# tylerlum/Vine_Robot_IsaacGymEnvs

Measured on NVIDIA B200. Metric: env-steps/s (whole box, device-timed), higher is better.
Workload: dtype f32

## Files before the change

### vine_robot_isaacgymenvs_b200/csrc/vine_b200.cu

```cuda
#include <cuda_runtime.h>
#include <stdio.h>
#include <stdlib.h>

#include "vine_device.cuh"
#include "vine_launch.cuh"

#define VINE_BLOCK 128
#ifndef VINE_STEP_MIN_BLOCKS
#define VINE_STEP_MIN_BLOCKS 0
#endif
#ifndef VINE_STEP_MIN_BLOCKS_CONTACT
#define VINE_STEP_MIN_BLOCKS_CONTACT 12
#endif
#define VINE_DBG_W 28

struct StepArgs {
  int64_t n, gid0;
  int64_t first, end;
  uint32_t k0, k1;
  float4 *S0, *S1, *S2, *S3, *S4, *S5;
  float2* ring;
  uint32_t* ctr;
  const float2* actions;
  float* obs; float* obs_clamped; float* rew;
// ... 186 lines not shown
  const bool noisy = p.randomize && p.obs_noise != 0.f;
  if (noisy) {
#pragma unroll
    for (uint32_t b = 0; b < VINE_MAX_OBS / 4; ++b) {
      if ((int)(4 * b) < p.O) normal4(philox4x32(a.k0, a.k1, E.gid, VINE_SITE_OBS_NOISE, E.step, b), &noise[4 * b]);
    }
  }
  PostOut o;
  post_physics(p, in, noisy ? noise : nullptr, o);
  agg = __fadd_rn(agg, o.rew);

  a.S0[e] = make_float4(q[0], q[1], q[2], q[3]);
  a.S1[e] = make_float4(q[4], q[5], qd[0], qd[1]);
  a.S2[e] = make_float4(qd[2], qd[3], qd[4], qd[5]);
  a.S3[e] = make_float4(E.smoothed, E.prev_cart_vel, E.prev_err, E.lip);
  a.S4[e] = make_float4(tip_y, tip_z, cart_body_vy, agg);
  if (E.reset_in) a.S5[e] = make_float4(target[1], target[2], obj[0], obj[1]);
  if (p.D > 0) a.ring[(int64_t)(E.step % (uint32_t)p.D) * a.n + e] = make_float2(E.new_rail, E.new_fpam);
  a.ctr[e] = E.step + 1u;
  a.rew[e] = o.rew;
  a.reset[e] = o.reset;
  a.progress[e] = progress;
  a.timeout[e] = o.timeout;
#pragma unroll
  for (int i = 0; i < VINE_MAX_OBS; ++i) if (i < p.O) row[i] = o.obs[i];
  if (a.dbg) {
    float* dbg = a.dbg + e * VINE_DBG_W;
    dbg[0] = E.u_rail; dbg[1] = E.u_fpam; dbg[2] = in.prev_u_rail; dbg[3] = E.rail_force;
    dbg[4] = tipvel_y; dbg[5] = tipvel_z;
    dbg[19] = cart_y_body;
#pragma unroll
    for (int i = 0; i < VINE_NUM_REWARDS; ++i) dbg[6 + i] = o.r[i];
#pragma unroll
    for (int i = 0; i < 6; ++i) dbg[20 + i] = div_rn(__fsub_rn(in.q[i], in.prev_q[i]), p.control_dt);
    dbg[26] = div_rn(__fsub_rn(in.tip[1], in.prev_tip[1]), p.control_dt);
    dbg[27] = div_rn(__fsub_rn(in.tip[2], in.prev_tip[2]), p.control_dt);
  }
}

#ifndef VINE_BLOCK_CONTACT
#define VINE_BLOCK_CONTACT 32
#endif

__device__ __forceinline__ void store_obs_rows_scattered(const VineParams& p, const StepArgs& a, const float* s_obs, int64_t mine) {
  const int lane = threadIdx.x & 31, w0 = threadIdx.x & ~31;
#pragma unroll 1
  for (int r = 0; r < 32; ++r) {
    const int64_t er = __shfl_sync(0xffffffffu, mine, r);
    if (er >= 0 && lane < p.O) {
      const float v = s_obs[(w0 + r) * (VINE_MAX_OBS + 1) + lane];
      a.obs[er * p.O + lane] = v;
      if (a.obs_clamped) a.obs_clamped[er * p.O + lane] = fminf(fmaxf(v, -p.clip_obs), p.clip_obs);
    }
  }
}

__device__ __forceinline__ int64_t slot_env(const StepArgs& a, int64_t slot) {
  if (!a.list) return a.first + slot;
  return (int64_t)(a.list_reversed ? a.list[a.n - 1 - slot] : a.list[slot]);
}

template <bool CONTACT>
__global__ void __launch_bounds__(CONTACT ? VINE_BLOCK_CONTACT : VINE_BLOCK, CONTACT ? VINE_STEP_MIN_BLOCKS_CONTACT : VINE_STEP_MIN_BLOCKS)
vine_step_kernel(const __grid_constant__ VineParams p, const StepArgs a) {
  vine_launch::grid_dependency_sync();
  constexpr int BLOCK = CONTACT ? VINE_BLOCK_CONTACT : VINE_BLOCK;
  __shared__ float s_obs[BLOCK * (VINE_MAX_OBS + 1)];
  __shared__ ContactScratch s_contact[CONTACT ? BLOCK / 32 : 1];
  ContactScratch* cs = &s_contact[CONTACT ? threadIdx.x >> 5 : 0];
  const int64_t count = a.list_count ? (int64_t)*a.list_count : a.end - a.first;
  const int lanes = (CONTACT && a.list && count <= (int64_t)gridDim.x * 8) ? 8 : BLOCK;
#pragma unroll 1
  for (int64_t base = (int64_t)blockIdx.x * lanes; base < count; base += (int64_t)gridDim.x * lanes) {
    const int64_t slot = base + threadIdx.x;
    const bool live = slot < count && (int)threadIdx.x < lanes;
    const bool ghost = CONTACT && !live;
    const int64_t e = live ? slot_env(a, slot) : (ghost ? slot_env(a, base) : -1);
    if (live || ghost) {
      EnvStep E; Dyn d;
      env_begin(p, a, e, E, d);
      Obstacles ob = {0, -1, 0.f, 0.f, 0.f, 0.f};
      ContactCache cc = {0u, ghost ? -1e30f : 1e30f, 0u};
      if (CONTACT) { const float4 s5 = a.S5[e]; build_obstacles(p, s5.x, s5.y, s5.z, s5.w, cs, ob); }
      const float m00inv = rcp_approx(fmaf(p.h, p.damping, p.mtot));
#pragma unroll 1
      for (int i = 0; i < p.C; ++i) {
        JointImp J;
        env_sim_step_begin(p, a, i, E, d, J);
#pragma unroll 1
        for (int s = 0; s < p.S; ++s) substep<CONTACT>(p, J, m00inv, E.rail_force, ob, cs, cc, d, E.lip, ghost);
      }
      if (!ghost) {
        env_end(p, a, e, E, d, s_obs + threadIdx.x * (VINE_MAX_OBS + 1));
        if (CONTACT && a.near) a.near[e] = cc.seen != 0u;
      }
    }
    __syncthreads();
    if (CONTACT && a.list) store_obs_rows_scattered(p, a, s_obs, live ? e : -1);
    else store_obs_block<BLOCK>(s_obs, p.O, a.first + base - (int64_t)blockIdx.x * BLOCK, a.end, p.clip_obs, a.obs, a.obs_clamped);
    __syncthreads();
  }
}

__global__ void __launch_bounds__(VINE_BLOCK) vine_step_far_kernel(const __grid_constant__ VineParams p, const StepArgs a) {
  __shared__ float s_obs[VINE_BLOCK * (VINE_MAX_OBS + 1)];
  const int64_t count = a.list_count ? a.n - (int64_t)*a.list_count : a.n;
  const int64_t slot = (int64_t)blockIdx.x * VINE_BLOCK + threadIdx.x;
  if ((int64_t)blockIdx.x * VINE_BLOCK >= count) return;
  const bool live = slot < count;
  int64_t e = live ? slot_env(a, slot) : -1;
  if (live) {
    EnvStep E; Dyn d;
    env_begin(p, a, e, E, d);
    Obstacles ob;
    { const float4 s5 = a.S5[e]; obstacle_bbox(p, s5.x, s5.y, s5.z, s5.w, ob); }
    float gap = chain_obstacle_gap(p, ob, d);
    bool given_up = !(gap > 0.f);
    float disp = -gap;
    ContactCache cc = {0u, 0.f, 0u};
    const float m00inv = rcp_approx(fmaf(p.h, p.damping, p.mtot));
#pragma unroll 1
    for (int i = 0; i < p.C && !given_up; ++i) {
      JointImp J;
      env_sim_step_begin(p, a, i, E, d, J);
#pragma unroll 1
      for (int s = 0; s < p.S; ++s) {
        substep<false>(p, J, m00inv, E.rail_force, ob, nullptr, cc, d, E.lip);
        disp += chain_displacement_bound(p, d);
        if (disp > p.cull_slack) {
          gap = chain_obstacle_gap(p, ob, d);
          if (!(gap > 0.f)) { given_up = true; break; }
          disp = -gap;
        }
      }
      E.lip = 0.f;
    }
    if (given_up) {
      a.redo_list[atomicAdd(a.redo_count, 1)] = (int32_t)e;
      e = -1;
    } else {
      env_end(p, a, e, E, d, s_obs + threadIdx.x * (VINE_MAX_OBS + 1));
      a.near[e] = 0;
    }
  }
  __syncthreads();
  store_obs_rows_scattered(p, a, s_obs, e);
}

__global__ void __launch_bounds__(1024) vine_bin_kernel(const StepArgs a) {
  __shared__ int s_near[32], s_far[32], s_base[2];
  const int64_t e = (int64_t)blockIdx.x * 1024 + threadIdx.x;
  const bool valid = e < a.n, nr = valid && a.near[e] != 0;
  const unsigned bn = __ballot_sync(0xffffffffu, nr), bf = __ballot_sync(0xffffffffu, valid && !nr);
  const int lane = threadIdx.x & 31, warp = threadIdx.x >> 5;
  if (lane == 0) { s_near[warp] = __popc(bn); s_far[warp] = __popc(bf); }
  __syncthreads();
  if (warp == 0) {
    const int cn = s_near[lane], cf = s_far[lane];
    int in = cn, jf = cf;
#pragma unroll
    for (int off = 1; off < 32; off <<= 1) {
      const int tn = __shfl_up_sync(0xffffffffu, in, off), tf = __shfl_up_sync(0xffffffffu, jf, off);
      if (lane >= off) { in += tn; jf += tf; }
    }
    s_near[lane] = in - cn; s_far[lane] = jf - cf;
    if (lane == 31) { s_base[0] = atomicAdd(a.bin_cursor, in); s_base[1] = atomicAdd(a.bin_cursor + 1, jf); }
  }
  __syncthreads();
  if (!valid) return;
  const unsigned lt = (1u << lane) - 1u;
  if (nr) a.perm[s_base[0] + s_near[warp] + __popc(bn & lt)] = (int32_t)e;
  else a.perm[a.n - 1 - (s_base[1] + s_far[warp] + __popc(bf & lt))] = (int32_t)e;
}

__global__ void vine_init_kernel(const __grid_constant__ VineParams p, const StepArgs a) {
  const int64_t e = (int64_t)blockIdx.x * blockDim.x + threadIdx.x;
  if (e >= a.n) return;
  uint32_t u[12];
  for (uint32_t b = 0; b < 3; ++b) {
    const uint4 r = philox4x32(a.k0, a.k1, (uint32_t)(a.gid0 + e), VINE_SITE_RESET, 0x40000000u, b);
    u[4 * b] = r.x; u[4 * b + 1] = r.y; u[4 * b + 2] = r.z; u[4 * b + 3] = r.w;
  }
  float target[3]; sample_targets(p, u, target);
  const float4 z = make_float4(0.f, 0.f, 0.f, 0.f);
  a.S0[e] = z; a.S1[e] = z; a.S2[e] = z; a.S3[e] = z;
  a.S4[e] = make_float4(p.tip0_y, p.tip0_z, 0.f, 0.f);
  a.S5[e] = make_float4(target[1], target[2], 0.f, 0.f);
  for (int k = 0; k < p.D; ++k) a.ring[(int64_t)k * a.n + e] = make_float2(0.f, 0.f);
  a.ctr[e] = 0u;
}

__global__ void vine_reset_idx_kernel(const __grid_constant__ VineParams p, const StepArgs a, const int64_t* ids, int64_t n_ids) {
  const int64_t i = (int64_t)blockIdx.x * blockDim.x + threadIdx.x;
  if (i >= n_ids) return;
  const int64_t e = ids[i];
  if (e < 0 || e >= a.n) return;
  float q[6], qd[6], target[3], obj[2];
  const float4 s5 = a.S5[e];
  target[0] = 0.f; target[1] = s5.x; target[2] = s5.y; obj[0] = s5.z; obj[1] = s5.w;
  reset_env(p, a.k0, a.k1, (uint32_t)(a.gid0 + e), a.ctr[e] | 0x80000000u, q, qd, target, obj);
  float4 s3 = a.S3[e], s4 = a.S4[e];
  s3.z = 0.f;
  s4.w = 0.f;
  if (!p.stale) {
    Dyn d; rel_to_abs(q, qd, d);
    float vy, vz; tip_fk(d, s4.x, s4.y, vy, vz);
    s4.z = 0.f; s3.w = 0.f; s3.y = 0.f;
  }
  a.S0[e] = make_float4(q[0], q[1], q[2], q[3]);
  a.S1[e] = make_float4(q[4], q[5], 0.f, 0.f);
// ... 80 lines not shown
  in.u_rail = io.u_rail_velocity[e]; in.prev_u_rail = io.prev_u_rail_velocity[e];
  for (int i = 0; i < VINE_MAX_CFI; ++i) in.contact[i] = (io.contact_force_norms && i < p.C) ? io.contact_force_norms[(int64_t)i * n + e] : 0.f;
  in.reset_in = io.reset_buf_in[e]; in.progress = io.progress_buf[e];
  float noise[VINE_MAX_OBS];
  const bool noisy = p.randomize && io.obs_noise != nullptr;
  if (noisy) for (int i = 0; i < p.O; ++i) noise[i] = io.obs_noise[(int64_t)p.O * e + i];
  PostOut o;
  post_physics(p, in, noisy ? noise : nullptr, o);
  for (int i = 0; i < p.O; ++i) io.obs_buf[(int64_t)p.O * e + i] = o.obs[i];
  io.rew_buf[e] = o.rew;
  if (io.reward_matrix) for (int i = 0; i < VINE_NUM_REWARDS; ++i) io.reward_matrix[VINE_NUM_REWARDS * e + i] = o.r[i];
  io.reset_buf_out[e] = o.reset;
  io.timeout_buf[e] = o.timeout;
}

__global__ void vine_pre_physics_kernel(const __grid_constant__ VineParams p, int64_t n, const VinePrePhysicsIO io) {
  const int64_t e = (int64_t)blockIdx.x * blockDim.x + threadIdx.x;
  if (e >= n) return;
  float a0 = io.actions[2 * e], a1 = io.actions[2 * e + 1];
  if (p.randomize && io.action_noise) {
    a0 = __fadd_rn(a0, __fmul_rn(p.act_noise, io.action_noise[2 * e]));
    a1 = __fadd_rn(a1, __fmul_rn(p.act_noise, io.action_noise[2 * e + 1]));
  }
  float u_rail, u_fpam;
  rescale_actions(p, a0, a1, u_rail, u_fpam);
  if (p.D > 0) {
    const float* hi = io.history_in + (int64_t)2 * p.D * e;
    float* ho = io.history_out + (int64_t)2 * p.D * e;
    const float o_rail = hi[0], o_fpam = hi[1];
    for (int k = 0; k + 1 < p.D; ++k) { ho[2 * k] = hi[2 * k + 2]; ho[2 * k + 1] = hi[2 * k + 3]; }
    ho[2 * (p.D - 1)] = u_rail; ho[2 * (p.D - 1) + 1] = u_fpam;
    u_rail = o_rail; u_fpam = o_fpam;
  }
  float s = io.smoothed_in[e];
  apply_overrides_and_smooth(p, u_rail, u_fpam, s);
  io.u_rail_velocity[e] = u_rail; io.u_fpam[e] = u_fpam; io.smoothed_out[e] = s;
}

__global__ void vine_actuation_kernel(const __grid_constant__ VineParams p, int64_t n, const VineActuationIO io) {
  const int64_t e = (int64_t)blockIdx.x * blockDim.x + threadIdx.x;
  if (e >= n) return;
  JointLaw law; joint_law_unscaled(law);
  if (io.dynamics_scaling) {
    const float* s = io.dynamics_scaling + 20 * e;
    for (int j = 0; j < VINE_NL; ++j) {
      law.K[j] = __fmul_rn(law.K[j], s[4 * j]); law.Cd[j] = __fmul_rn(law.Cd[j], s[4 * j + 1]);
      law.b[j] = __fmul_rn(law.b[j], s[4 * j + 2]); law.B[j] = __fmul_rn(law.B[j], s[4 * j + 3]);
    }
  }
  float pv = io.prev_cart_vel[e], pe = io.prev_cart_vel_error[e];
  io.dof_efforts[6 * e] = rail_controller(p, io.cart_vel_y[e], io.u_rail_velocity[e],
                                          io.accel_scaling ? io.accel_scaling[e] : 1.f, pv, pe);
  for (int j = 0; j < VINE_NL; ++j)
    io.dof_efforts[6 * e + j + 1] = joint_torque(law, j, io.dof_pos[6 * e + j + 1], io.dof_vel[6 * e + j + 1], io.u_fpam_to_use[e]);
  io.prev_cart_vel_out[e] = pv; io.prev_cart_vel_error_out[e] = pe;
}

template <bool CONTACT>
__global__ void __launch_bounds__(VINE_BLOCK) vine_simulate_kernel(const __grid_constant__ VineParams p, int64_t n, const VineSimulateIO io) {
  __shared__ ContactScratch s_contact[CONTACT ? VINE_BLOCK / 32 : 1];
  ContactScratch* cs = &s_contact[CONTACT ? threadIdx.x >> 5 : 0];
  const int64_t e0 = (int64_t)blockIdx.x * blockDim.x + threadIdx.x;
  const bool ghost = e0 >= n;
  if (ghost && !CONTACT) return;
  const int64_t e = ghost ? n - 1 : e0;
  float q[6], qd[6], efforts[6];
  for (int i = 0; i < 6; ++i) { q[i] = io.dof_pos[6 * e + i]; qd[i] = io.dof_vel[6 * e + i]; efforts[i] = io.dof_efforts[6 * e + i]; }
  JointLaw law; joint_law_unscaled(law);
  if (io.dynamics_scaling) {
    const float* s = io.dynamics_scaling + 20 * e;
    for (int j = 0; j < VINE_NL; ++j) {
      law.K[j] = __fmul_rn(law.K[j], s[4 * j]); law.Cd[j] = __fmul_rn(law.Cd[j], s[4 * j + 1]);
      law.b[j] = __fmul_rn(law.b[j], s[4 * j + 2]); law.B[j] = __fmul_rn(law.B[j], s[4 * j + 3]);
    }
  }
  const float u_use = io.u_fpam_to_use ? io.u_fpam_to_use[e] : 0.f;
  Obstacles ob = {0, -1, 0.f, 0.f, 0.f, 0.f};
  ContactCache cc = {0u, ghost ? -1e30f : 1e30f, 0u};
  if (CONTACT) build_obstacles(p, io.target_positions[3 * e + 1], io.target_positions[3 * e + 2],
                               io.object_info[2 * e], io.object_info[2 * e + 1], cs, ob);
  Dyn d; rel_to_abs(q, qd, d);
  JointImp J; joint_implicit_consts(p, law, u_use, efforts, J);
  float lip = 0.f;
  const float m00inv = rcp_approx(fmaf(p.h, p.damping, p.mtot));
#pragma unroll 1
  for (int s = 0; s < p.S; ++s) substep<CONTACT>(p, J, m00inv, efforts[0], ob, cs, cc, d, lip, ghost);
  if (ghost) return;
  float ty, tz, vy, vz; tip_fk(d, ty, tz, vy, vz);
  abs_to_rel(d, q, qd);
  for (int i = 0; i < 6; ++i) { io.dof_pos[6 * e + i] = q[i]; io.dof_vel[6 * e + i] = qd[i]; }
  if (io.tip_positions) { io.tip_positions[3 * e] = 0.f; io.tip_positions[3 * e + 1] = ty; io.tip_positions[3 * e + 2] = tz; }
  if (io.tip_velocities) { io.tip_velocities[3 * e] = 0.f; io.tip_velocities[3 * e + 1] = vy; io.tip_velocities[3 * e + 2] = vz; }
  if (io.shelf_contact_force) io.shelf_contact_force[e] = lip;
}

__global__ void vine_philox_kernel(uint32_t k0, uint32_t k1, uint32_t gid, uint32_t site, uint32_t step, uint32_t block0,
                                   int64_t n_blocks, uint32_t* out) {
  const int64_t i = (int64_t)blockIdx.x * blockDim.x + threadIdx.x;
  if (i >= n_blocks) return;
  const uint4 r = philox4x32(k0, k1, gid, site, step, block0 + (uint32_t)i);
  out[4 * i] = r.x; out[4 * i + 1] = r.y; out[4 * i + 2] = r.z; out[4 * i + 3] = r.w;
}

__global__ void vine_gae_kernel(const float* __restrict__ rewards, const float* __restrict__ values,
                                const float* __restrict__ dones, const float* __restrict__ last_values,
                                const float* __restrict__ last_dones, int64_t T, int64_t N, float gamma, float gt,
                                float* __restrict__ adv, float* __restrict__ ret) {
  vine_launch::grid_dependency_sync();
  const int64_t e = (int64_t)blockIdx.x * blockDim.x + threadIdx.x;
  if (e >= N) return;
  float nextv = last_values[e], nonterm = __fsub_rn(1.0f, last_dones[e]), lastgaelam = 0.f;
  float r = rewards[(T - 1) * N + e], v = values[(T - 1) * N + e], dn = dones[(T - 1) * N + e];
  for (int64_t t = T - 1; t >= 0; --t) {
    float r2 = 0.f, v2 = 0.f, d2 = 0.f;
    if (t > 0) { r2 = rewards[(t - 1) * N + e]; v2 = values[(t - 1) * N + e]; d2 = dones[(t - 1) * N + e]; }
    const float delta = __fsub_rn(__fadd_rn(r, __fmul_rn(__fmul_rn(gamma, nextv), nonterm)), v);
    lastgaelam = __fadd_rn(delta, __fmul_rn(__fmul_rn(gt, nonterm), lastgaelam));
    adv[t * N + e] = lastgaelam;
    ret[t * N + e] = __fadd_rn(lastgaelam, v);
    nextv = v; nonterm = __fsub_rn(1.0f, dn);
    r = r2; v = v2; dn = d2;
  }
}

static inline unsigned grid_for(int64_t n, int block) { return (unsigned)((n + block - 1) / block); }

extern "C" {

int vine_abi_version(void) { return VINE_ABI_VERSION; }

int vine_set_programmatic_launch(int enabled) {
  const int before = vine_launch::programmatic_launch_enabled();
  vine_launch::programmatic_launch_enabled() = enabled ? 1 : 0;
  return before;
}

int vine_config_defaults(VineConfig* c) {
  if (!c) return VINE_ERR_INVALID_ARG;
  memset(c, 0, sizeof(*c));
  c->struct_size = (int32_t)sizeof(*c);
  c->substeps = 10; c->dt = 0.00833; c->gravity_z = -9.81;
  c->control_freq_inv = 4; c->max_episode_length = 500;
  c->clip_observations = 5.0; c->clip_actions = 1.0;
  c->observation_type = VINE_OBS_POS_AND_FD_VEL_AND_OBJ_INFO; c->scale_observations = 1;
  c->create_shelf = 0; c->create_pipe = 1;
  c->use_smoothed_fpam = 1; c->action_delay = 1;
  c->smoothing_alpha_inflate = 0.81; c->smoothing_alpha_deflate = 0.86;
  c->fpam_min = -0.1; c->fpam_max = 3.0; c->rail_velocity_scale = 1.0;
  c->damping = 2e-2; c->stiffness = 0.0;
  c->rail_soft_limit = 0.3; c->rail_p_gain = 10.0; c->rail_d_gain = 0.0; c->rail_acceleration = 8.0;
  c->randomize_dof_init = 1; c->randomize_targets = 1;
  c->random_init_cart_min_y = -0.1 * 0.3; c->random_init_cart_max_y = 0.3;
  c->success_dist = 0.08;
  c->min_target_depth_in_obstacle = -0.05; c->max_target_depth_in_obstacle = 0.2;
  c->min_target_y = -0.48; c->max_target_y = -0.4; c->min_target_z = 0.58; c->max_target_z = 0.67;
  const double w[VINE_NUM_REWARDS] = {0, 0, 1, 0, 0.1, 0, 0, 0, 0, 1, 0, 0, 0.10};
  memcpy(c->reward_weights, w, sizeof(w));
  c->use_target_reached_reset = 1;
  c->vine_randomize = 1;
  c->dynamics_scaling_min = 0.999; c->dynamics_scaling_max = 1.001;
  c->accel_target_scaling_min = 1.0; c->accel_target_scaling_max = 1.0;
  c->torque_law_integration = VINE_TORQUE_LAW_IMPLICIT;
  c->emulate_stale_body_state = 1;
  c->revolute_lower = -3.4e38; c->revolute_upper = 3.4e38;
  c->prismatic_lower = -3.4e38; c->prismatic_upper = 3.4e38;
  c->contact_stiffness = 2000.0; c->contact_damping = 2.0; c->contact_rest_offset = 0.001;
  c->contact_cull_slack = 0.01; c->contact_binning = 1;
  return VINE_OK;
}
// ... 350 lines not shown
```

### vine_robot_isaacgymenvs_b200/csrc/vine_device.cuh

```cuda
#pragma once
#include <cuda_runtime.h>

#include "vine_params.h"

#define VDEV __device__ __forceinline__

VDEV uint4 philox4x32(uint32_t k0, uint32_t k1, uint32_t c0, uint32_t c1, uint32_t c2, uint32_t c3) {
#pragma unroll
  for (int r = 0; r < 10; ++r) {
    const uint32_t hi0 = __umulhi(0xD2511F53u, c0), lo0 = 0xD2511F53u * c0;
    const uint32_t hi1 = __umulhi(0xCD9E8D57u, c2), lo1 = 0xCD9E8D57u * c2;
    c0 = hi1 ^ c1 ^ k0; c1 = lo1; c2 = hi0 ^ c3 ^ k1; c3 = lo0;
    k0 += 0x9E3779B9u; k1 += 0xBB67AE85u;
  }
  return make_uint4(c0, c1, c2, c3);
}

VDEV float rcp_approx(float x) { float r; asm("rcp.approx.ftz.f32 %0, %1;" : "=f"(r) : "f"(x)); return r; }
VDEV float sin_approx(float x) { float r; asm("sin.approx.ftz.f32 %0, %1;" : "=f"(r) : "f"(x)); return r; }
VDEV float cos_approx(float x) { float r; asm("cos.approx.ftz.f32 %0, %1;" : "=f"(r) : "f"(x)); return r; }
VDEV float div_rn(float a, float b) {
  const bool bypass = a == 0.f && fabsf(b) > 0.f && fabsf(b) < __int_as_float(0x7f800000);
  const float q = __fdiv_rn(bypass ? 1.f : a, b);
  return bypass ? __int_as_float(__float_as_int(a) ^ (__float_as_int(b) & (int)0x80000000)) : q;
// ... 305 lines not shown
#pragma unroll
    for (int j = 0; j < VINE_NL; ++j) {
      const float lw = VINE_LINK_LEN * d.v[j + 1];
      vy = fmaf(-lw, d.C[j], vy); vz = fmaf(-lw, d.S[j], vz);
      ch[32 * (CH_PY + j + 1)] = py[j + 1]; ch[32 * (CH_PZ + j + 1)] = pz[j + 1];
      ch[32 * (CH_VY + j + 1)] = vy; ch[32 * (CH_VZ + j + 1)] = vz;
      ch[32 * (CH_S + j)] = d.S[j]; ch[32 * (CH_C + j)] = d.C[j]; ch[32 * (CH_W + j)] = d.v[j + 1];
    }
  }
  const int cnt = __popc(pm);
  const unsigned below = (1u << lane) - 1u;
  int next = 0, total = 0;
#pragma unroll
  for (int k = 0; k < 5; ++k) {
    const unsigned plane = __ballot_sync(0xffffffffu, (cnt >> k) & 1);
    next += __popc(plane & below) << k;
    total += __popc(plane) << k;
  }
  unsigned todo = pm, toadd = pm;
  int next_add = next;
  float lfy = 0.f, lfz = 0.f;
#pragma unroll 1
  for (int base = 0; base < total; base += VINE_PAIR_PASS) {
    while (todo && next < base + VINE_PAIR_PASS) {
      const int b = __ffs(todo) - 1;
      todo &= todo - 1;
      cs->item[next - base] = (unsigned short)(lane | (b << 5));
      ++next;
    }
    __syncwarp();
    const int n_pass = min(VINE_PAIR_PASS, total - base);
#pragma unroll 1
    for (int i = lane; i < n_pass; i += 32) {
      const int it = cs->item[i];
      PairLoad L;
      pair_load(p, cs, it & 31, it >> 5, L);
      cs->res[i][0] = L.fy; cs->res[i][1] = L.fz; cs->res[i][2] = L.t;
    }
    __syncwarp();
    while (toadd && next_add < base + VINE_PAIR_PASS) {
      const int b = __ffs(toadd) - 1;
      toadd &= toadd - 1;
      const float* rs = cs->res[next_add - base];
      ++next_add;
      const float Lfy = rs[0], Lfz = rs[1], Lt = rs[2];
      if (Lfy != 0.f || Lfz != 0.f) {
        const int r = b / 5, j = b - 5 * r;
        f[0] += Lfy;
#pragma unroll
        for (int m = 0; m < VINE_NL; ++m) {
          const float q = m == j ? Lt : (py[m + 1] - py[m]) * Lfz - (pz[m + 1] - pz[m]) * Lfy;
          if (m <= j) f[m + 1] += q;
        }
        if (r == ob.lip) { lfy -= Lfy; lfz -= Lfz; }
      }
    }
    __syncwarp();
  }
  const float l2 = lfy * lfy + lfz * lfz;
  const float l = sqrtf(l2 > 0.f ? l2 : 1.f);
  return l2 > 0.f ? l : 0.f;
}

struct JointImp { float kk[VINE_NL], ek[VINE_NL], tc[VINE_NL], gam[VINE_NL], diag[VINE_NL]; };

VDEV void joint_implicit_consts(const VineParams& p, const JointLaw& law, float u_use, const float efforts[6], JointImp& J) {
#pragma unroll
  for (int j = 0; j < VINE_NL; ++j) {
    float dd;
    if (p.implicit_law) {
      J.kk[j] = p.stiffness + law.K[j]; dd = p.damping + law.Cd[j];
      J.tc[j] = -fmaf(law.B[j], u_use, law.b[j]);
    } else {
      J.kk[j] = p.stiffness; dd = p.damping; J.tc[j] = efforts[j + 1];
    }
    J.ek[j] = fmaf(p.h, J.kk[j], dd);
    J.gam[j] = fmaf(p.h, dd, p.h * p.h * J.kk[j]) + p.armature;
  }
#pragma unroll
  for (int j = 0; j < VINE_NL; ++j) J.diag[j] = p.alpha[j] + J.gam[j] + (j + 1 < VINE_NL ? J.gam[j + 1] : 0.f);
}

template <bool CONTACT>
VDEV void substep(const VineParams& p, const JointImp& J, float m00inv, float rail_force, const Obstacles& ob,
                  ContactScratch* cs, ContactCache& cc, Dyn& d, float& lip, bool ghost = false) {
  float a[VINE_NL], b[VINE_NL], As[VINE_NL], Bs[VINE_NL];
#pragma unroll
  for (int j = 0; j < VINE_NL; ++j) { const float w2 = __fmul_rn(d.v[j + 1], d.v[j + 1]); a[j] = __fmul_rn(d.C[j], w2); b[j] = __fmul_rn(d.S[j], w2); }
  As[VINE_NL - 2] = __fmul_rn(p.Lbeta[VINE_NL - 1], a[VINE_NL - 1]);
  Bs[VINE_NL - 2] = __fmul_rn(p.Lbeta[VINE_NL - 1], b[VINE_NL - 1]);
#pragma unroll
  for (int j = VINE_NL - 3; j >= 0; --j) {
    As[j] = __fmaf_rn(p.Lbeta[j + 1], a[j + 1], As[j + 1]);
    Bs[j] = __fmaf_rn(p.Lbeta[j + 1], b[j + 1], Bs[j + 1]);
  }
  float f[6];
  f[0] = __fmaf_rn(-p.inv_L, __fmaf_rn(p.Lbeta[0], b[0], Bs[0]), __fmaf_rn(-p.damping, d.v[0], rail_force));
  {
    float Ap = a[0], Bp = b[0];
    f[1] = __fmaf_rn(d.C[0], Bs[0], __fmul_rn(d.S[0], __fsub_rn(p.gbeta[0], As[0])));
#pragma unroll
    for (int j = 1; j < VINE_NL; ++j) {
      const float P = j == VINE_NL - 1 ? __fmul_rn(p.Lbeta[j], Ap) : __fmaf_rn(p.Lbeta[j], Ap, As[j]);
      const float Q = j == VINE_NL - 1 ? __fmul_rn(p.Lbeta[j], Bp) : __fmaf_rn(p.Lbeta[j], Bp, Bs[j]);
      f[j + 1] = __fmaf_rn(d.C[j], Q, __fmul_rn(d.S[j], __fsub_rn(p.gbeta[j], P)));
      if (j + 1 < VINE_NL) { Ap = __fadd_rn(Ap, a[j]); Bp = __fadd_rn(Bp, b[j]); }
    }
  }
  {
    float tn = 0.f;
#pragma unroll
    for (int j = VINE_NL - 1; j >= 0; --j) {
      const float th = j == 0 ? d.x[1] : __fsub_rn(d.x[j + 1], d.x[j]);
      const float thd = j == 0 ? d.v[1] : __fsub_rn(d.v[j + 1], d.v[j]);
      const float t = __fmaf_rn(-J.ek[j], thd, __fmaf_rn(-J.kk[j], th, J.tc[j]));
      f[j + 1] = __fadd_rn(f[j + 1], j == VINE_NL - 1 ? t : __fsub_rn(t, tn));
      tn = t;
    }
  }
  if constexpr (CONTACT) lip = contact_forces(p, ob, cs, cc, d, f, ghost);
  float M[6][6];
#pragma unroll
  for (int j = 0; j < VINE_NL; ++j) {
    M[j + 1][0] = __fmul_rn(-p.beta[j], d.C[j]);
    M[j + 1][j + 1] = J.diag[j];
#pragma unroll
    for (int m = 0; m < j; ++m) {
      const float c = __fmaf_rn(d.C[j], d.C[m], __fmul_rn(d.S[j], d.S[m]));
      M[j + 1][m + 1] = (m == j - 1) ? __fmaf_rn(p.Lbeta[j], c, -J.gam[j]) : __fmul_rn(p.Lbeta[j], c);
    }
  }
  float dinv[6];
  dinv[0] = m00inv;
#pragma unroll
  for (int j = 1; j < 6; ++j) {
    float u[5];
    float dj = M[j][j];
#pragma unroll
    for (int q = 0; q < j; ++q) {
      float uq = M[j][q];
#pragma unroll
      for (int r = 0; r < q; ++r) uq = __fmaf_rn(-u[r], M[q][r], uq);
      u[q] = uq;
      const float l = __fmul_rn(uq, dinv[q]);
      M[j][q] = l;
      dj = __fmaf_rn(-uq, l, dj);
    }
    dinv[j] = rcp_approx(dj);
  }
#pragma unroll
  for (int i = 1; i < 6; ++i)
#pragma unroll
    for (int q = 0; q < i; ++q) f[i] = __fmaf_rn(-M[i][q], f[q], f[i]);
#pragma unroll
  for (int i = 0; i < 6; ++i) f[i] = __fmul_rn(f[i], dinv[i]);
#pragma unroll
  for (int i = 4; i >= 0; --i)
#pragma unroll
    for (int q = i + 1; q < 6; ++q) f[i] = __fmaf_rn(-M[q][i], f[q], f[i]);
  d.v[0] = __fmaf_rn(p.h, f[0], d.v[0]); d.x[0] = __fmaf_rn(p.h, d.v[0], d.x[0]);
#pragma unroll
  for (int j = 0; j < VINE_NL; ++j) {
    d.v[j + 1] = __fmaf_rn(p.h, f[j + 1], d.v[j + 1]);
    d.x[j + 1] = __fmaf_rn(p.h, d.v[j + 1], d.x[j + 1]);
    link_trig(d.x[j + 1], d.S[j], d.C[j]);
  }
}

VDEV float norm3_torch(float x, float y, float z) {
  return __fsqrt_rn(__fmaf_rn(z, z, __fmaf_rn(y, y, __fmul_rn(x, x))));
}

struct PostIn {
  float q[6], qd[6], prev_q[6];
  float tip[3], prev_tip[3], tipvel[3], target[3], target_vel[3], obj[2];
  float cart_y, smoothed, u_fpam, u_rail, prev_u_rail;
  float contact[VINE_MAX_CFI];
  int64_t reset_in, progress;
};

struct PostOut { float obs[VINE_MAX_OBS]; float rew; float r[VINE_NUM_REWARDS]; int64_t reset; unsigned char timeout; };

VDEV void observation_row(const VineParams& p, const PostIn& in, float raw[VINE_MAX_OBS]) {
  float fdq[6], fdt[3];
#pragma unroll
  for (int i = 0; i < 6; ++i) fdq[i] = div_rn(__fsub_rn(in.q[i], in.prev_q[i]), p.control_dt);
#pragma unroll
  for (int i = 0; i < 3; ++i) fdt[i] = div_rn(__fsub_rn(in.tip[i], in.prev_tip[i]), p.control_dt);
  const int t = p.obs_type;
#pragma unroll
  for (int i = 0; i < VINE_MAX_OBS; ++i) raw[i] = 0.f;
  if (t == VINE_OBS_TIP_AND_CART_AND_OBJ_INFO) {
    raw[0] = in.q[0]; raw[1] = fdq[0];
#pragma unroll
    for (int i = 0; i < 3; ++i) { raw[2 + i] = in.tip[i]; raw[5 + i] = fdt[i]; raw[8 + i] = in.target[i]; raw[11 + i] = in.target_vel[i]; }
    raw[14] = in.smoothed; raw[15] = in.prev_u_rail; raw[16] = in.obj[0]; raw[17] = in.obj[1];
    return;
  }
#pragma unroll
  for (int i = 0; i < 6; ++i) raw[i] = in.q[i];
  if (t != VINE_OBS_POS_ONLY) {
#pragma unroll
    for (int i = 0; i < 6; ++i) raw[6 + i] = t == VINE_OBS_POS_AND_VEL ? in.qd[i] : (t == VINE_OBS_POS_AND_PREV_POS ? in.prev_q[i] : fdq[i]);
  }
  if (t == VINE_OBS_POS_ONLY) {
#pragma unroll
    for (int i = 0; i < 3; ++i) { raw[6 + i] = in.tip[i]; raw[9 + i] = in.target[i]; }
    raw[12] = in.smoothed; raw[13] = in.prev_u_rail;
    return;
  }
#pragma unroll
  for (int i = 0; i < 3; ++i) {
    raw[12 + i] = in.tip[i];
    raw[15 + i] = t == VINE_OBS_POS_AND_VEL ? in.tipvel[i] : (t == VINE_OBS_POS_AND_PREV_POS ? in.prev_tip[i] : fdt[i]);
    raw[18 + i] = in.target[i]; raw[21 + i] = in.target_vel[i];
  }
  raw[24] = in.smoothed; raw[25] = in.prev_u_rail;
  if (t == VINE_OBS_POS_AND_FD_VEL_AND_OBJ_INFO) { raw[26] = in.obj[0]; raw[27] = in.obj[1]; }
}

VDEV void post_physics(const VineParams& p, const PostIn& in, const float* noise, PostOut& o) {
  float raw[VINE_MAX_OBS];
  observation_row(p, in, raw);
#pragma unroll
  for (int i = 0; i < VINE_MAX_OBS; ++i) {
    float v = div_rn(raw[i], p.obs_scale[i]);
    if (noise != nullptr && i < p.O) v = __fadd_rn(v, __fmul_rn(p.obs_noise, noise[i]));
    o.obs[i] = v;
  }
  const float dist = norm3_torch(__fsub_rn(in.tip[0], in.target[0]), __fsub_rn(in.tip[1], in.target[1]),
                                 __fsub_rn(in.tip[2], in.target[2]));
  const bool reached = dist < p.success_dist;
  const bool limit_hit = (in.cart_y > p.soft_limit) || (in.cart_y < -p.soft_limit);
  const bool tip_limit_hit = in.tip[1] < in.target[1];
  float contact = 0.f; bool nonzero = false;
  if (p.shelf) {
    float s = in.contact[0];
#pragma unroll
    for (int i = 1; i < VINE_MAX_CFI; ++i) if (i < p.C) s = __fadd_rn(s, in.contact[i]);
    contact = div_rn(s, (float)p.C);
    nonzero = contact > 0.f;
  }
// ... 71 lines not shown
```

### vine_robot_isaacgymenvs_b200/csrc/vine_params.h

```cpp
#pragma once
#include <math.h>
#include <stdint.h>
#include <string.h>

#include "../../include/vine_b200.h"

#define VINE_NL 5
#define VINE_MAX_OBS 28
#define VINE_MAX_CFI 8
#define VINE_MAX_RECTS 5

enum { VINE_SITE_ACTION_NOISE = 1, VINE_SITE_DYNAMICS = 2, VINE_SITE_OBS_NOISE = 3, VINE_SITE_RESET = 4 };

struct VineParams {
  int O, C, S, D;
  int obs_type, scaled;
  int shelf, pipe;
  int use_smoothed, force_fpam, force_rail;
  int randomize, implicit_law, stale;
  int rand_dof_init, rand_targets;
  int reach_reset, tip_reset, contact_reset;
  int64_t max_len_m1;
  float clip_act, clip_obs, act_noise, obs_noise;
  float rail_scale, fpam_range, fpam_min, alpha_inf, alpha_def;
  float dt, control_dt, rail_force_max, rail_accel, p_gain, d_gain;
  float dyn_min, dyn_rng, acc_min, acc_rng;
  float cull_slack;
  float soft_limit, success_dist;
  float w[VINE_NUM_REWARDS];
  float obs_scale[VINE_MAX_OBS];
  float rev_lo, rev_rng, cart_lo, cart_rng, ty_lo, ty_rng, tz_lo, tz_rng, dep_lo, dep_rng;
  float ty_hi, tz_lo_fixed;
  float h, g, damping, stiffness, armature;
  float kc, dc, rest;
  float beta[VINE_NL], alpha[VINE_NL], mtot;
  float Lbeta[VINE_NL], gbeta[VINE_NL], inv_L;
  float tip0_y, tip0_z;
};

static const double kLinkLen = 0.0885, kLinkCom = 0.04425, kCartMass = 0.4, kBaseAngle = 3.1415;
static const double kPivotZ = 1.0 - 0.025 - 0.01;
static const double kLinkMass[VINE_NL] = {0.005, 0.005, 0.005, 0.005, 0.1};
static const double kLinkInertia[VINE_NL] = {6.89246e-6, 6.89246e-6, 6.89246e-6, 6.89246e-6, 1.01559e-4};
#define VINE_LINK_LEN 0.0885f
#define VINE_BASE_ANGLE 3.1415f
#define VINE_PIVOT_Z 0.965f
#define VINE_LINK_RADIUS 0.0381f
#define VINE_FPAM_RADIUS 0.0169f
#define VINE_FPAM_OFFSET 0.055f

static const float kObsScale28[28] = {0.12f, 0.269f, 0.148f, 0.249f, 0.148f, 0.344f, 0.67f, 2.22f, 1.47f, 1.14f,
                                      0.903f, 0.716f, 0.0656f, 0.238f, 0.0656f, 0.732f, 2.0f, 0.732f, 0.02f,
                                      0.0235f, 0.02f, 0.732f, 2.0f, 0.732f, 0.845f, 0.86f, 0.0385f, 0.5f};
static const float kObsScale18[18] = {0.12f, 0.67f, 0.0656f, 0.238f, 0.0656f, 0.732f, 2.0f, 0.732f, 0.02f, 0.0235f,
                                      0.02f, 0.732f, 2.0f, 0.732f, 0.845f, 0.86f, 0.0385f, 0.5f};

static inline int vine_obs_width(int t) {
  switch (t) {
    case VINE_OBS_POS_ONLY: return 14;
    case VINE_OBS_POS_AND_VEL:
    case VINE_OBS_POS_AND_FD_VEL:
    case VINE_OBS_POS_AND_PREV_POS: return 26;
    case VINE_OBS_POS_AND_FD_VEL_AND_OBJ_INFO: return 28;
    case VINE_OBS_TIP_AND_CART_AND_OBJ_INFO: return 18;
    default: return -1;
  }
}

static inline int vine_derive_params(const VineConfig* c, VineParams* p, const char** why) {
  *why = "";
  if (c->struct_size != (int32_t)sizeof(VineConfig)) { *why = "VineConfig.struct_size mismatch"; return VINE_ERR_ABI_MISMATCH; }
  memset(p, 0, sizeof(*p));
  p->O = vine_obs_width(c->observation_type);
  if (p->O < 0) { *why = "unknown OBSERVATION_TYPE"; return VINE_ERR_INVALID_ARG; }
  p->C = c->control_freq_inv; p->S = c->substeps; p->D = c->action_delay;
  if (p->C < 1 || p->C > VINE_MAX_CFI) { *why = "controlFrequencyInv must be in 1..8"; return VINE_ERR_INVALID_ARG; }
  if (p->S < 1) { *why = "sim.substeps must be >= 1"; return VINE_ERR_INVALID_ARG; }
  if (p->D < 0 || p->D > VINE_MAX_ACTION_DELAY) { *why = "ACTION_DELAY must be in 0..8"; return VINE_ERR_INVALID_ARG; }
  if (!(c->dt > 0)) { *why = "sim.dt must be > 0"; return VINE_ERR_INVALID_ARG; }
  p->obs_type = c->observation_type; p->scaled = c->scale_observations != 0;
  for (int i = 0; i < VINE_MAX_OBS; ++i) p->obs_scale[i] = 1.0f;
  if (p->scaled) {
    if (c->observation_type == VINE_OBS_POS_AND_FD_VEL_AND_OBJ_INFO) memcpy(p->obs_scale, kObsScale28, sizeof(kObsScale28));
    else if (c->observation_type == VINE_OBS_TIP_AND_CART_AND_OBJ_INFO) memcpy(p->obs_scale, kObsScale18, sizeof(kObsScale18));
    else { *why = "Observation scaling not implemented for this OBSERVATION_TYPE (V5:267-268)"; return VINE_ERR_UNSUPPORTED; }
  }
  p->shelf = c->create_shelf != 0; p->pipe = c->create_pipe != 0;
  p->use_smoothed = c->use_smoothed_fpam != 0; p->force_fpam = c->force_u_fpam != 0; p->force_rail = c->force_u_rail_velocity != 0;
  p->randomize = c->vine_randomize != 0;
  p->implicit_law = c->torque_law_integration == VINE_TORQUE_LAW_IMPLICIT;
  p->stale = c->emulate_stale_body_state != 0;
  p->rand_dof_init = c->randomize_dof_init != 0; p->rand_targets = c->randomize_targets != 0;
  p->reach_reset = c->use_target_reached_reset != 0; p->tip_reset = c->use_tip_limit_hit_reset != 0;
  p->contact_reset = c->use_nonzero_contact_force_reset != 0;
  p->max_len_m1 = (int64_t)c->max_episode_length - 1;
  p->clip_act = (float)c->clip_actions; p->clip_obs = (float)c->clip_observations;
  p->act_noise = (float)c->action_noise_std; p->obs_noise = (float)c->observation_noise_std;
  p->rail_scale = (float)c->rail_velocity_scale;
  p->fpam_range = (float)(c->fpam_max - c->fpam_min); p->fpam_min = (float)c->fpam_min;
  p->alpha_inf = (float)c->smoothing_alpha_inflate; p->alpha_def = (float)c->smoothing_alpha_deflate;
  p->dt = (float)c->dt; p->control_dt = (float)(c->dt * (double)c->control_freq_inv);
  p->rail_force_max = (float)(c->rail_acceleration / 2.0); p->rail_accel = (float)c->rail_acceleration;
  p->p_gain = (float)c->rail_p_gain; p->d_gain = (float)c->rail_d_gain;
  p->dyn_min = (float)c->dynamics_scaling_min; p->dyn_rng = (float)c->dynamics_scaling_max - p->dyn_min;
  p->acc_min = (float)c->accel_target_scaling_min; p->acc_rng = (float)c->accel_target_scaling_max - p->acc_min;
  p->soft_limit = (float)c->rail_soft_limit; p->success_dist = (float)c->success_dist;
  for (int i = 0; i < VINE_NUM_REWARDS; ++i) p->w[i] = (float)c->reward_weights[i];
  {
    const double ten = 10.0 * 3.14159265358979323846 / 180.0;
    float lo = (float)fmax(c->revolute_lower, -ten), hi = (float)fmin(c->revolute_upper, ten);
    p->rev_lo = lo; p->rev_rng = hi - lo;
    lo = (float)fmax(c->prismatic_lower, c->random_init_cart_min_y); hi = (float)fmin(c->prismatic_upper, c->random_init_cart_max_y);
    p->cart_lo = lo; p->cart_rng = hi - lo;
  }
  p->ty_lo = (float)c->min_target_y; p->ty_rng = (float)c->max_target_y - p->ty_lo; p->ty_hi = (float)c->max_target_y;
  p->tz_lo = (float)c->min_target_z; p->tz_rng = (float)c->max_target_z - p->tz_lo; p->tz_lo_fixed = p->tz_lo;
  p->dep_lo = (float)c->min_target_depth_in_obstacle; p->dep_rng = (float)c->max_target_depth_in_obstacle - p->dep_lo;
  p->h = (float)(c->dt / (double)c->substeps); p->g = (float)(-c->gravity_z);
  p->damping = (float)c->damping; p->stiffness = (float)c->stiffness; p->armature = (float)c->armature;
  p->kc = (float)c->contact_stiffness; p->dc = (float)c->contact_damping; p->rest = (float)c->contact_rest_offset;
  double tail = 0;
  for (int j = VINE_NL - 1; j >= 0; --j) {
    p->beta[j] = (float)(kLinkLen * tail + kLinkCom * kLinkMass[j]);
    p->alpha[j] = (float)(kLinkInertia[j] + kLinkMass[j] * kLinkCom * kLinkCom + kLinkLen * kLinkLen * tail);
    tail += kLinkMass[j];
  }
  p->mtot = (float)(kCartMass + tail);
  for (int j = 0; j < VINE_NL; ++j) { p->Lbeta[j] = (float)kLinkLen * p->beta[j]; p->gbeta[j] = p->g * p->beta[j]; }
  p->inv_L = (float)(1.0 / kLinkLen);
  p->tip0_y = (float)(-5.0 * kLinkLen * sin(kBaseAngle)); p->tip0_z = (float)(kPivotZ + 5.0 * kLinkLen * cos(kBaseAngle));
  return VINE_OK;
}
```

Baseline: 2.109 billion.

## Eliminate cart DOF analytically via Schur complement in substep linear solve

The cart row and column are removed from the 6x6 implicit mass-matrix LDL solve. A Schur complement reduces it to a 5x5 system over the links, using host-precomputed constants (m00inv, kap, mb2) that fold the cart mass, damping and the coupling terms. The cart acceleration is then recovered by back-substitution. This trims FLOPs and registers in the hot substep loop, at the cost of slightly different floating-point rounding from the reformulated algebra.

Measured after the change: 2.153 billion (median of 6 runs). 2.1% higher.

```diff
diff --git a/vine_robot_isaacgymenvs_b200/csrc/vine_b200.cu b/vine_robot_isaacgymenvs_b200/csrc/vine_b200.cu
--- a/vine_robot_isaacgymenvs_b200/csrc/vine_b200.cu
+++ b/vine_robot_isaacgymenvs_b200/csrc/vine_b200.cu
@@ -292,13 +292,12 @@
       Obstacles ob = {0, -1, 0.f, 0.f, 0.f, 0.f};
       ContactCache cc = {0u, ghost ? -1e30f : 1e30f, 0u};
       if (CONTACT) { const float4 s5 = a.S5[e]; build_obstacles(p, s5.x, s5.y, s5.z, s5.w, cs, ob); }
-      const float m00inv = rcp_approx(fmaf(p.h, p.damping, p.mtot));
 #pragma unroll 1
       for (int i = 0; i < p.C; ++i) {
         JointImp J;
         env_sim_step_begin(p, a, i, E, d, J);
 #pragma unroll 1
-        for (int s = 0; s < p.S; ++s) substep<CONTACT>(p, J, m00inv, E.rail_force, ob, cs, cc, d, E.lip, ghost);
+        for (int s = 0; s < p.S; ++s) substep<CONTACT>(p, J, E.rail_force, ob, cs, cc, d, E.lip, ghost);
       }
       if (!ghost) {
         env_end(p, a, e, E, d, s_obs + threadIdx.x * (VINE_MAX_OBS + 1));
@@ -328,14 +327,13 @@
     bool given_up = !(gap > 0.f);
     float disp = -gap;
     ContactCache cc = {0u, 0.f, 0u};
-    const float m00inv = rcp_approx(fmaf(p.h, p.damping, p.mtot));
 #pragma unroll 1
     for (int i = 0; i < p.C && !given_up; ++i) {
       JointImp J;
       env_sim_step_begin(p, a, i, E, d, J);
 #pragma unroll 1
       for (int s = 0; s < p.S; ++s) {
-        substep<false>(p, J, m00inv, E.rail_force, ob, nullptr, cc, d, E.lip);
+        substep<false>(p, J, E.rail_force, ob, nullptr, cc, d, E.lip);
         disp += chain_displacement_bound(p, d);
         if (disp > p.cull_slack) {
           gap = chain_obstacle_gap(p, ob, d);
@@ -582,9 +580,8 @@
   Dyn d; rel_to_abs(q, qd, d);
   JointImp J; joint_implicit_consts(p, law, u_use, efforts, J);
   float lip = 0.f;
-  const float m00inv = rcp_approx(fmaf(p.h, p.damping, p.mtot));
 #pragma unroll 1
-  for (int s = 0; s < p.S; ++s) substep<CONTACT>(p, J, m00inv, efforts[0], ob, cs, cc, d, lip, ghost);
+  for (int s = 0; s < p.S; ++s) substep<CONTACT>(p, J, efforts[0], ob, cs, cc, d, lip, ghost);
   if (ghost) return;
   float ty, tz, vy, vz; tip_fk(d, ty, tz, vy, vz);
   abs_to_rel(d, q, qd);
diff --git a/vine_robot_isaacgymenvs_b200/csrc/vine_device.cuh b/vine_robot_isaacgymenvs_b200/csrc/vine_device.cuh
--- a/vine_robot_isaacgymenvs_b200/csrc/vine_device.cuh
+++ b/vine_robot_isaacgymenvs_b200/csrc/vine_device.cuh
@@ -411,7 +411,7 @@
 }
 
 template <bool CONTACT>
-VDEV void substep(const VineParams& p, const JointImp& J, float m00inv, float rail_force, const Obstacles& ob,
+VDEV void substep(const VineParams& p, const JointImp& J, float rail_force, const Obstacles& ob,
                   ContactScratch* cs, ContactCache& cc, Dyn& d, float& lip, bool ghost = false) {
   float a[VINE_NL], b[VINE_NL], As[VINE_NL], Bs[VINE_NL];
 #pragma unroll
@@ -448,22 +448,28 @@
     }
   }
   if constexpr (CONTACT) lip = contact_forces(p, ob, cs, cc, d, f, ghost);
-  float M[6][6];
+  float bc[VINE_NL], kc[VINE_NL - 1];
+  {
+    const float ty = __fmul_rn(p.m00inv, f[0]);
+#pragma unroll
+    for (int j = 0; j < VINE_NL; ++j) { bc[j] = __fmul_rn(p.beta[j], d.C[j]); f[j + 1] = __fmaf_rn(bc[j], ty, f[j + 1]); }
+  }
+#pragma unroll
+  for (int k = 0; k < VINE_NL - 1; ++k) kc[k] = __fmul_rn(p.kap[k], d.C[k]);
+  float M[VINE_NL][VINE_NL];
 #pragma unroll
   for (int j = 0; j < VINE_NL; ++j) {
-    M[j + 1][0] = __fmul_rn(-p.beta[j], d.C[j]);
-    M[j + 1][j + 1] = J.diag[j];
+    M[j][j] = __fmaf_rn(-p.mb2[j], __fmul_rn(d.C[j], d.C[j]), J.diag[j]);
 #pragma unroll
     for (int m = 0; m < j; ++m) {
-      const float c = __fmaf_rn(d.C[j], d.C[m], __fmul_rn(d.S[j], d.S[m]));
-      M[j + 1][m + 1] = (m == j - 1) ? __fmaf_rn(p.Lbeta[j], c, -J.gam[j]) : __fmul_rn(p.Lbeta[j], c);
-    }
-  }
-  float dinv[6];
-  dinv[0] = m00inv;
-#pragma unroll
-  for (int j = 1; j < 6; ++j) {
-    float u[5];
+      const float c = __fmaf_rn(d.C[j], kc[m], __fmul_rn(d.S[j], d.S[m]));
+      M[j][m] = (m == j - 1) ? __fmaf_rn(p.Lbeta[j], c, -J.gam[j]) : __fmul_rn(p.Lbeta[j], c);
+    }
+  }
+  float dinv[VINE_NL];
+#pragma unroll
+  for (int j = 0; j < VINE_NL; ++j) {
+    float u[VINE_NL - 1];
     float dj = M[j][j];
 #pragma unroll
     for (int q = 0; q < j; ++q) {
@@ -478,15 +484,18 @@
     dinv[j] = rcp_approx(dj);
   }
 #pragma unroll
-  for (int i = 1; i < 6; ++i)
-#pragma unroll
-    for (int q = 0; q < i; ++q) f[i] = __fmaf_rn(-M[i][q], f[q], f[i]);
-#pragma unroll
-  for (int i = 0; i < 6; ++i) f[i] = __fmul_rn(f[i], dinv[i]);
-#pragma unroll
-  for (int i = 4; i >= 0; --i)
-#pragma unroll
-    for (int q = i + 1; q < 6; ++q) f[i] = __fmaf_rn(-M[q][i], f[q], f[i]);
+  for (int i = 1; i < VINE_NL; ++i)
+#pragma unroll
+    for (int q = 0; q < i; ++q) f[i + 1] = __fmaf_rn(-M[i][q], f[q + 1], f[i + 1]);
+#pragma unroll
+  for (int i = 0; i < VINE_NL; ++i) f[i + 1] = __fmul_rn(f[i + 1], dinv[i]);
+#pragma unroll
+  for (int i = VINE_NL - 2; i >= 0; --i)
+#pragma unroll
+    for (int q = i + 1; q < VINE_NL; ++q) f[i + 1] = __fmaf_rn(-M[q][i], f[q + 1], f[i + 1]);
+#pragma unroll
+  for (int j = 0; j < VINE_NL; ++j) f[0] = __fmaf_rn(bc[j], f[j + 1], f[0]);
+  f[0] = __fmul_rn(p.m00inv, f[0]);
   d.v[0] = __fmaf_rn(p.h, f[0], d.v[0]); d.x[0] = __fmaf_rn(p.h, d.v[0], d.x[0]);
 #pragma unroll
   for (int j = 0; j < VINE_NL; ++j) {
diff --git a/vine_robot_isaacgymenvs_b200/csrc/vine_params.h b/vine_robot_isaacgymenvs_b200/csrc/vine_params.h
--- a/vine_robot_isaacgymenvs_b200/csrc/vine_params.h
+++ b/vine_robot_isaacgymenvs_b200/csrc/vine_params.h
@@ -33,8 +33,11 @@
   float ty_hi, tz_lo_fixed;
   float h, g, damping, stiffness, armature;
   float kc, dc, rest;
-  float beta[VINE_NL], alpha[VINE_NL], mtot;
+  float beta[VINE_NL], alpha[VINE_NL];
   float Lbeta[VINE_NL], gbeta[VINE_NL], inv_L;
+  float m00inv;
+  float kap[VINE_NL];
+  float mb2[VINE_NL];
   float tip0_y, tip0_z;
 };
 
@@ -119,15 +122,21 @@
   p->h = (float)(c->dt / (double)c->substeps); p->g = (float)(-c->gravity_z);
   p->damping = (float)c->damping; p->stiffness = (float)c->stiffness; p->armature = (float)c->armature;
   p->kc = (float)c->contact_stiffness; p->dc = (float)c->contact_damping; p->rest = (float)c->contact_rest_offset;
-  double tail = 0;
+  double tail = 0, beta[VINE_NL];
   for (int j = VINE_NL - 1; j >= 0; --j) {
-    p->beta[j] = (float)(kLinkLen * tail + kLinkCom * kLinkMass[j]);
+    beta[j] = kLinkLen * tail + kLinkCom * kLinkMass[j];
+    p->beta[j] = (float)beta[j];
     p->alpha[j] = (float)(kLinkInertia[j] + kLinkMass[j] * kLinkCom * kLinkCom + kLinkLen * kLinkLen * tail);
     tail += kLinkMass[j];
   }
-  p->mtot = (float)(kCartMass + tail);
   for (int j = 0; j < VINE_NL; ++j) { p->Lbeta[j] = (float)kLinkLen * p->beta[j]; p->gbeta[j] = p->g * p->beta[j]; }
   p->inv_L = (float)(1.0 / kLinkLen);
+  const double m00inv = 1.0 / (kCartMass + tail + c->dt / (double)c->substeps * c->damping);
+  p->m00inv = (float)m00inv;
+  for (int j = 0; j < VINE_NL; ++j) {
+    p->kap[j] = (float)(1.0 - m00inv * beta[j] / kLinkLen);
+    p->mb2[j] = (float)(m00inv * beta[j] * beta[j]);
+  }
   p->tip0_y = (float)(-5.0 * kLinkLen * sin(kBaseAngle)); p->tip0_z = (float)(kPivotZ + 5.0 * kLinkLen * cos(kBaseAngle));
   return VINE_OK;
 }
```
